# facebookresearch/dmc-net

Measured on AMD Instinct MI355X. Metric: clips/sec (3-seg 224x224) DMC-gen+ResNet-18 train step, higher is better.
Workload: dtype f32

## Files before the change

dmc-net_amd/csrc/conv_x3q.hip:

```cpp
#include "dmc_common.h"
#include "x3s_common.h"
#include <type_traits>
#include <utility>

using namespace dmc;
using namespace dmc::x3;

namespace {

constexpr int QBM = 256, QBN = 64;
constexpr int QWSLOT = 3 * QBN * 32;
constexpr int QWB = 3 * QWSLOT;
constexpr int QEP = 272, QETILE = 32 * QEP;

template <int NW_, int NPB_, int NT_>
struct QG {
    static constexpr int NW = NW_, NPB = NPB_, NT = NT_;
    static constexpr int NA = NW / 2;
    static constexpr int KP = (NT + NA - 1) / NA;
    static constexpr int PT = 3 * KP;
    static constexpr int KW = (18 + NA - 1) / NA;
    static constexpr int ZROW = 32 * NT;
    static constexpr int PSL = (ZROW + 1) * 32;
    static constexpr int PB = 3 * PSL;
// ... 165 lines not shown
            if (U < total_units) {
#pragma unroll
                for (int i = 0; i < QPT; ++i) dma_patch(U / NUNIT, std::integral_constant<int, U % NUNIT>{}, U, i);
            }
        });
    } else {
        static_for<2>([&](auto gc) {
            constexpr int g = decltype(gc)::value;
            if (g < total_steps) {
#pragma unroll
                for (int i = 0; i < KW; ++i) dma_weight(g / NSTEP, std::integral_constant<int, g % NSTEP>{}, g, wq + NA * i);
            }
        });
    }
    asm volatile("s_waitcnt vmcnt(0)" ::: "memory");
    __builtin_amdgcn_s_barrier();

    Frag F0, F1;
    int pb = 0, wb = 0;
    int xcur[NSH];
#pragma unroll
    for (int sh = 0; sh < NSH; ++sh) xcur[sh] = xaddr[sh];
    int wcur = waddr;
    {
        constexpr int sh0 = P::STEP[0].s[0].sh;
        load_frags(F0, xcur[sh0], wcur, std::integral_constant<int, 0>{});
    }

    auto frag_of = [&](auto ic) -> Frag& {
        if constexpr (decltype(ic)::value == 0) return F0; else return F1;
    };
#pragma unroll 1
    for (int c = 0; c < nchunk; ++c) {
        static_for<NSTEP>([&](auto jc) {
            constexpr int J = decltype(jc)::value;
            constexpr int JN = (J + 1) % NSTEP;
            constexpr int unit = P::STEP[J].unit, nslot = P::STEP[J].nslot;
            constexpr bool unit_last = (P::STEP[JN].unit != unit) || (NUNIT == 1 && J == NSTEP - 1);
            constexpr int par = slots_before<P>(J) & 1;
            const int g = c * NSTEP + J, U = c * NUNIT + unit;
            static_for<nslot - 1>([&](auto kc) {
                constexpr int k = decltype(kc)::value;
                constexpr int sh_next = P::STEP[J].s[k + 1].sh, acc_k = P::STEP[J].s[k].acc;
                load_frags(frag_of(std::integral_constant<int, (par + k + 1) & 1>{}), xcur[sh_next], wcur, std::integral_constant<int, k + 1>{});
                mfma_slot(frag_of(std::integral_constant<int, (par + k) & 1>{}), std::integral_constant<int, acc_k>{}, nothing);
                interleave();
            });
            if (GEO::COUNTED && grp_a && U + 2 < total_units) asm volatile("s_waitcnt vmcnt(%0) lgkmcnt(0)" :: "n"(QPT) : "memory");
            else asm volatile("s_waitcnt vmcnt(0) lgkmcnt(0)" ::: "memory");
            __builtin_amdgcn_s_barrier();
            const int pb_old = pb, wb_old = wb;
            if constexpr (unit_last) {
                pb = pb == QNPB - 1 ? 0 : pb + 1;
#pragma unroll
                for (int sh = 0; sh < NSH; ++sh) xcur[sh] = xaddr[sh] + pb * QPB;
            }
            wb ^= 1;
            wcur = waddr + wb * QWB;
            constexpr int kl = nslot - 1;
            constexpr int sh_first = P::STEP[JN].s[0].sh, acc_last = P::STEP[J].s[kl].acc;
            if (g + 1 < total_steps)
                load_frags(frag_of(std::integral_constant<int, (par + kl + 1) & 1>{}), xcur[sh_first], wcur, std::integral_constant<int, 0>{});
            constexpr int J2 = (J + 2) % NSTEP, C2 = (J + 2) / NSTEP;
            constexpr int U3 = (unit + QNPB) % NUNIT, CU3 = (unit + QNPB) / NUNIT;
            const bool wgo = !grp_a && g + 2 < total_steps;
            const bool pgo = grp_a && unit_last && U + QNPB < total_units;
            mfma_slot(frag_of(std::integral_constant<int, (par + kl) & 1>{}), std::integral_constant<int, acc_last>{}, [&](int p) {
                if (wgo) {
#pragma unroll
                    for (int i = p; i < KW; i += 6) dma_weight(c + C2, std::integral_constant<int, J2>{}, wb_old, wq + NA * i);
                }
                if constexpr (unit_last) {
                    if (pgo) {
#pragma unroll
                        for (int i = p; i < QPT; i += 6) dma_patch(c + CU3, std::integral_constant<int, U3>{}, pb_old, i);
                    }
                }
            });
        });
    }

    __syncthreads();
    constexpr int CW = 32 * TN, LPR = CW / 4, RPI = 64 / LPR;
    char* etile = lds_q + wave * QETILE;
    const int mw0 = m0 + wm * 32;
    const int rbase = blockIdx.y * QBN + wn * CW;
    const bool ok = mw0 + l31 <= mlast;
#pragma unroll
    for (int A = 0; A < NACC; ++A) {
#pragma unroll
        for (int j = 0; j < TN; ++j)
#pragma unroll
            for (int g4 = 0; g4 < 4; ++g4) {
                float4 v = make_float4(acc[A][j][4 * g4], acc[A][j][4 * g4 + 1], acc[A][j][4 * g4 + 2], acc[A][j][4 * g4 + 3]);
                if (!ok) v = make_float4(0.f, 0.f, 0.f, 0.f);
                *reinterpret_cast<float4*>(etile + l31 * QEP + (32 * j + 8 * g4 + 4 * khalf) * 4) = v;
            }
        float* const yout = (NACC == 2 && A == 1) ? a.y1 : a.y0;
#pragma unroll
        for (int it = 0; it < 32 / RPI; ++it) {
            const int prow = RPI * it + lane / LPR;
            const int m = mw0 + prow;
            const float4 v = *reinterpret_cast<const float4*>(etile + prow * QEP + (lane % LPR) * 16);
            if (m <= mlast) {
                size_t opix = (size_t)m;
                if (NACC == 4) {
                    const int n = m / HW, rem = m - n * HW, ya = rem / a.W, xb = rem - ya * a.W;
                    opix = ((size_t)n * (2 * a.H) + 2 * ya + (A >> 1)) * (2 * a.W) + 2 * xb + (A & 1);
                }
                *reinterpret_cast<float4*>(yout + opix * a.R + rbase + (lane % LPR) * 4) = v;
            }
        }
        if (NACC == 2) {
            double* const part = A == 1 ? a.part1 : a.part0;
            if (part) {
                double* red = reinterpret_cast<double*>(lds_q + QNW * QETILE);
                if (lane < CW) {
                    double d1 = 0.0, d2 = 0.0;
#pragma unroll 8
                    for (int p = 0; p < 32; ++p) {
                        const double v = (double)*reinterpret_cast<const float*>(etile + p * QEP + lane * 4);
                        d1 += v;
                        d2 += v * v;
                    }
                    red[(wm * 64 + wn * CW + lane) * 2 + 0] = d1;
                    red[(wm * 64 + wn * CW + lane) * 2 + 1] = d2;
                }
                __syncthreads();
                for (int cc = tid; cc < QBN; cc += QNW * 64) {
                    double e1 = 0.0, e2 = 0.0;
#pragma unroll
                    for (int w = 0; w < WM; ++w) { e1 += red[(w * 64 + cc) * 2 + 0]; e2 += red[(w * 64 + cc) * 2 + 1]; }
                    double* dst = part + ((size_t)blockIdx.x * a.R + blockIdx.y * QBN + cc) * 2;
                    dst[0] = e1; dst[1] = e2;
                }
                __syncthreads();
            }
        }
    }
}

__global__ __launch_bounds__(256) void x3q_pack_w_kernel(const float* __restrict__ w3, const float* __restrict__ w1,
                                                         unsigned short* __restrict__ wf, unsigned short* __restrict__ wt, int Cout, int Cin) {
    const bool transposed = blockIdx.y == 1;
    unsigned short* dst = transposed ? wt : wf;
    if (!dst) return;
    const int R = transposed ? Cin : Cout, K = transposed ? Cout : Cin;
    const int nchunk = K >> 4;
    const long total = (long)R * 10 * K;
    for (long i = (long)blockIdx.x * 256 + threadIdx.x; i < total; i += (long)gridDim.x * 256) {
        long t = i;
        const int kk = (int)(t & 15); t >>= 4;
        const int rl = (int)(t & 63); t >>= 6;
        const int slot = (int)(t % 10); t /= 10;
        const int ch = (int)(t % nchunk);
        const int rt = (int)(t / nchunk);
        const int r = rt * 64 + rl, k = ch * 16 + kk;
        constexpr int FWD_TAP[10] = {0, 2, 6, 8, 3, 5, 1, 7, 4, 9};
        const int tap = transposed ? slot : FWD_TAP[slot];
        const int co = transposed ? k : r, ci = transposed ? r : k;
        const float v = tap < 9 ? w3[((long)co * 9 + tap) * Cin + ci] : w1[(long)co * Cin + ci];
        unsigned u0, u1, u2;
        split3(v, u0, u1, u2);
        const size_t base = ((((size_t)(rt * nchunk + ch) * 10 + slot) * 3) * 64 + rl) * 16 + (kk ^ (((rl >> 3) & 1) << 3));
        dst[base] = (unsigned short)(u0 >> 16);
        dst[base + 64 * 16] = (unsigned short)(u1 >> 16);
        dst[base + 2 * 64 * 16] = (unsigned short)(u2 >> 16);
    }
}

__global__ __launch_bounds__(256) void x3q_split_kernel(const float* __restrict__ x, unsigned short* __restrict__ xq, int N, int H, int W, int C) {
    const int c8 = C >> 3, nchunk = C >> 4, H2 = H >> 1, W2 = W >> 1;
    const long total = (long)N * H * W * c8;
    const size_t Mq = (size_t)N * H2 * W2;
    for (long o = (long)blockIdx.x * 256 + threadIdx.x; o < total; o += (long)gridDim.x * 256) {
        const long m = o / c8;
        const int g = (int)(o - m * c8);
        const int xx = (int)(m % W), yy = (int)((m / W) % H), n = (int)(m / ((long)W * H));
        const float4 a = reinterpret_cast<const float4*>(x)[2 * o], b = reinterpret_cast<const float4*>(x)[2 * o + 1];
        const float v[8] = {a.x, a.y, a.z, a.w, b.x, b.y, b.z, b.w};
        const int cls = (yy & 1) * 2 + (xx & 1);
        x3s_store8(xq, v, Mq, 4 * nchunk, ((size_t)n * H2 + (yy >> 1)) * W2 + (xx >> 1), g + cls * 2 * nchunk);
    }
}

__global__ __launch_bounds__(256) void x3q_merge_kernel(const unsigned short* __restrict__ xq, float* __restrict__ x, int N, int H, int W, int C) {
    const int nchunk = C >> 4, H2 = H >> 1, W2 = W >> 1;
    const long total = (long)N * H * W * C;
    const size_t Mq = (size_t)N * H2 * W2, plane = Mq * 16;
    for (long o = (long)blockIdx.x * 256 + threadIdx.x; o < total; o += (long)gridDim.x * 256) {
        const long m = o / C;
        const int c = (int)(o - m * C);
        const int xx = (int)(m % W), yy = (int)((m / W) % H), n = (int)(m / ((long)W * H));
        const int cls = (yy & 1) * 2 + (xx & 1);
        const size_t mq = ((size_t)n * H2 + (yy >> 1)) * W2 + (xx >> 1);
        const size_t w = ((size_t)(cls * nchunk + (c >> 4)) * Mq + mq) * 16 + (c & 15);
        const float s0 = __uint_as_float((unsigned)xq[w] << 16);
        const float s1 = __uint_as_float((unsigned)xq[(size_t)4 * nchunk * plane + w] << 16);
        const float s2 = __uint_as_float((unsigned)xq[(size_t)8 * nchunk * plane + w] << 16);
        x[o] = (s0 + s1) + s2;
    }
}

int stream_blocks_q(long total) {
    long b = (total + 255) / 256;
    return (int)(b < 1 ? 1 : (b > 8192 ? 8192 : b));
}

int q_patch_pixels_max(long M, int W) {
// ... 488 lines not shown
```

dmc-net_amd/csrc/conv_x3s.hip:

```cpp
#include "dmc_common.h"
#include "x3s_common.h"
#include <type_traits>

using namespace dmc;
using namespace dmc::x3;

namespace {

__global__ __launch_bounds__(256) void x3s_split_kernel(const float* __restrict__ x, unsigned short* __restrict__ xs, long M, int C) {
    const int c8 = C >> 3;
    const long total = M * c8;
    const int nchunk = C >> 4;
    for (long o = (long)blockIdx.x * 256 + threadIdx.x; o < total; o += (long)gridDim.x * 256) {
        const long m = o / c8;
        const int g = (int)(o - m * c8);
        const float4 a = reinterpret_cast<const float4*>(x)[2 * o], b = reinterpret_cast<const float4*>(x)[2 * o + 1];
        const float v[8] = {a.x, a.y, a.z, a.w, b.x, b.y, b.z, b.w};
        x3s_store8(xs, v, (size_t)M, nchunk, (size_t)m, g);
    }
}

__global__ __launch_bounds__(256) void x3s_merge_kernel(const unsigned short* __restrict__ xs, float* __restrict__ x, long M, int C) {
    const long total = M * C;
    const size_t plane = (size_t)M * 16;
    const int nchunk = C >> 4;
    for (long o = (long)blockIdx.x * 256 + threadIdx.x; o < total; o += (long)gridDim.x * 256) {
        const long m = o / C;
        const int c = (int)(o - m * C);
        const size_t w = ((size_t)(c >> 4) * M + m) * 16 + (c & 15);
        const float a = __uint_as_float((unsigned)xs[w] << 16);
        const float b = __uint_as_float((unsigned)xs[(size_t)nchunk * plane + w] << 16);
        const float d = __uint_as_float((unsigned)xs[(size_t)2 * nchunk * plane + w] << 16);
        x[o] = (a + b) + d;
    }
}

__global__ __launch_bounds__(256) void x3s_pack_w_kernel(const float* __restrict__ w, unsigned short* __restrict__ wf,
                                                         unsigned short* __restrict__ wt, int Cout, int Cin, int mirror) {
    const bool transposed = blockIdx.y == 1;
    unsigned short* dst = transposed ? wt : wf;
    if (!dst) return;
    const int R = transposed ? Cin : Cout, K = transposed ? Cout : Cin;
    const int nchunk = K >> 4;
    const long total = (long)R * 9 * K;
    for (long i = (long)blockIdx.x * 256 + threadIdx.x; i < total; i += (long)gridDim.x * 256) {
        long t = i;
        const int kk = (int)(t & 15); t >>= 4;
        const int rl = (int)(t & 63); t >>= 6;
        const int tap = (int)(t % 9); t /= 9;
        const int ch = (int)(t % nchunk);
        const int rt = (int)(t / nchunk);
        const int r = rt * 64 + rl, k = ch * 16 + kk;
        const float v = transposed ? w[((long)k * 9 + (mirror ? 8 - tap : tap)) * Cin + r] : w[((long)r * 9 + tap) * Cin + k];
        unsigned u0, u1, u2;
        split3(v, u0, u1, u2);
        const size_t base = ((((size_t)(rt * nchunk + ch) * 9 + tap) * 3) * 64 + rl) * 16 + (kk ^ (((rl >> 3) & 1) << 3));
        dst[base] = (unsigned short)(u0 >> 16);
        dst[base + 64 * 16] = (unsigned short)(u1 >> 16);
        dst[base + 2 * 64 * 16] = (unsigned short)(u2 >> 16);
    }
}

struct X3Args {
    const void* xs;
    const void* wp;
    float* y;
    const float* addend;
    double* stat_part;
    int N, H, W, K, R;
    int M;
    unsigned plane_bytes;
    const float* bnb_y = nullptr;
    const float* bnb_stats = nullptr;
    const float* bnb_gamma = nullptr;
    const float* bnb_beta = nullptr;
    const unsigned char* bnb_mask = nullptr;
    int bnb_relu = 0;
    double* bnb_part = nullptr;
    int part_blocks = -1;
    int ablate;
};

template <int WM, int WN, int TM, int TN, int PPMAX, bool STAG = false, int CLS = 1>
__global__ __launch_bounds__(WM * WN * 64) void x3s_conv_kernel(X3Args a) {
    constexpr int NW = WM * WN, BM = 32 * TM * WM, BN = 32 * TN * WN;
    static_assert(BN == 64, "packed weight image is 64 rows wide");
    static_assert(PPMAX % 32 == 0 || PPMAX % 32 == 1, "patch transfers move 32 pixel rows");
    constexpr int PSL = PPMAX * 32;
    constexpr int PB = 3 * PSL;
    constexpr int WB = 3 * 3 * BN * 32;
    constexpr int WOFF = 2 * PB;
    static_assert(!STAG || NW >= 4, "two transfer groups need four waves");
    constexpr int NA = STAG ? NW / 2 : NW, NB = NW - (STAG ? NA : 0);
    constexpr int NDW = (PPMAX / 32 + NA - 1) / NA;
    constexpr int NEW = WB / 1024;
    constexpr int NEWW = (NEW + NB - 1) / NB;
    extern __shared__ __attribute__((aligned(1024))) char lds_x3[];

    const int tid = threadIdx.x, lane = tid & 63;
    const int wave = __builtin_amdgcn_readfirstlane(tid >> 6);
    const int wm = wave % WM, wn = wave / WM;
    const int l31 = lane & 31, khalf = lane >> 5;
    const unsigned lds0 = lds_addr_of(lds_x3);

    const int HW = a.H * a.W, PW = a.W;
    constexpr int ZROW = PPMAX - 1;
    const int m0 = blockIdx.x * BM;
    const int mlast = (m0 + BM < a.M ? m0 + BM : a.M) - 1;
    const int r_first = m0 / PW, r_last = mlast / PW;
    const int f0 = (r_first > 0 ? r_first - 1 : 0) * PW;
    const int f1 = (r_last + 2) * PW < a.M ? (r_last + 2) * PW : a.M;
    const int PP = f1 - f0;
    const int ND = (PP + 31) >> 5;

    unsigned pvoff[NDW];
#pragma unroll
    for (int k = 0; k < NDW; ++k) {
        const int pr = 32 * (wave + NA * k) + (lane >> 1), h = lane & 1;
        pvoff[k] = pr < PP ? (unsigned)(f0 + pr) * 32u + (unsigned)((h ^ ((pr >> 3) & 1)) << 4) : OOB;
    }
    int xaddr[TM][9];
#pragma unroll
    for (int i = 0; i < TM; ++i) {
        int m = m0 + (wm * TM + i) * 32 + l31;
        if (m > mlast) m = mlast;
        const int n = m / HW, rem = m - n * HW, yy = rem / a.W, xx = rem - yy * a.W;
        const int pp = m - f0;
#pragma unroll
        for (int t = 0; t < 9; ++t) {
            const int dx = CLS == 4 ? (t % 3 == 0 ? 1 : 0) : t % 3 - 1, dy = CLS == 4 ? (t / 3 == 0 ? 1 : 0) : t / 3 - 1;
            const int row = (xx + dx >= 0 && xx + dx < a.W && yy + dy >= 0 && yy + dy < a.H) ? pp + dy * PW + dx : ZROW;
            xaddr[i][t] = row * 32 + ((khalf ^ ((row >> 3) & 1)) << 4);
        }
    }
    const int waddr = (wn * TN * 32 + l31) * 32 + ((khalf ^ ((l31 >> 3) & 1)) << 4);

    const u32x4 srd_x = make_srd(a.xs);
    const int nchunk = a.K >> 4, S = 3 * nchunk;
    const u32x4 srd_w = make_srd(reinterpret_cast<const char*>(a.wp) + (size_t)blockIdx.y * S * WB);
    const unsigned lane16 = (unsigned)lane * 16u;

    const bool grp_a = wave < NA, grp_b = !STAG || wave >= NA;
    const int wb = STAG ? wave - NA : wave;
    auto dma_weight = [&](int step, int wbuf, int k) {
        const int e = wb + NB * k;
        if (e < NEW) dma_buf16(srd_w, lane16, (unsigned)(step * WB + e * 1024), lds0 + WOFF + wbuf * WB + e * 1024);
    };
    auto dma_patch = [&](int chunk, int slice, int pbuf, int k) {
        const int d = wave + NA * k;
        if (d < ND) dma_buf16(srd_x, pvoff[k], (unsigned)(slice * nchunk + chunk) * a.plane_bytes, lds0 + pbuf * PB + slice * PSL + d * 1024);
    };
    auto issue_weights = [&](int step, int wbuf) {
        if (grp_b) {
#pragma unroll
            for (int k = 0; k < NEWW; ++k) dma_weight(step, wbuf, k);
        }
    };
    auto issue_patch = [&](int chunk, int slice, int pbuf) {
        if (grp_a) {
#pragma unroll
            for (int k = 0; k < NDW; ++k) dma_patch(chunk, slice, pbuf, k);
        }
    };

    f32x16 acc[CLS][TM][TN];
#pragma unroll
// ... 40 lines not shown
        for (int k = 0; k < NRD; ++k) {
            __builtin_amdgcn_sched_group_barrier(0x008, 1, 0);
            __builtin_amdgcn_sched_group_barrier(0x100, 1, 0);
        }
        __builtin_amdgcn_sched_group_barrier(0x008, NMF - NRD, 0);
    };
    const bool dma_on = !(DMC_ABL(a.ablate) & 64);
    auto step = [&](auto pbufc, auto wbufc, auto qc, Frag& FA, Frag& FB, int c) {
        constexpr int pbuf = decltype(pbufc)::value, wbuf = decltype(wbufc)::value, q = decltype(qc)::value;
        using NP = std::integral_constant<int, q == 2 ? (pbuf ^ 1) : pbuf>;
        using NWB = std::integral_constant<int, wbuf ^ 1>;
        using NT = std::integral_constant<int, q == 2 ? 0 : 3 * (q + 1)>;
        using T0 = std::integral_constant<int, 3 * q>;
        using T1 = std::integral_constant<int, 3 * q + 1>;
        using T2 = std::integral_constant<int, 3 * q + 2>;
        const int s = 3 * c + q;
        load_frags(pbufc, wbufc, std::integral_constant<int, 3 * q + 1>{}, FB);
        if constexpr (STAG) {
            const bool go = grp_b && dma_on && s + 1 < S;
            mfma_frags(FA, T0{}, [&](int p) {
                if (go) {
#pragma unroll
                    for (int k = p; k < NEWW; k += 6) dma_weight(s + 1, wbuf ^ 1, k);
                }
            });
        } else {
            mfma_frags(FA, T0{}, nothing);
            interleave();
        }
        load_frags(pbufc, wbufc, std::integral_constant<int, 3 * q + 2>{}, FA);
        mfma_frags(FB, T1{}, nothing);
        interleave();
        if (DMC_ABL(a.ablate) & 16) asm volatile("s_waitcnt lgkmcnt(0)" ::: "memory");
        else asm volatile("s_waitcnt vmcnt(0) lgkmcnt(0)" ::: "memory");
        __builtin_amdgcn_s_barrier();
        const int vc = q == 2 ? c + 2 : c + 1;
        if constexpr (STAG) {
            if (s + 1 < S) load_frags(NP{}, NWB{}, NT{}, FB);
            const bool go = grp_a && dma_on && vc < nchunk;
            mfma_frags(FA, T2{}, [&](int p) {
                if (go) {
#pragma unroll
                    for (int k = p; k < NDW; k += 6) dma_patch(vc, q == 2 ? 0 : q + 1, q == 2 ? pbuf : (pbuf ^ 1), k);
                }
            });
        } else {
            if (dma_on) {
                if (s + 2 < S) issue_weights(s + 2, wbuf);
                if (vc < nchunk) issue_patch(vc, q == 2 ? 0 : q + 1, q == 2 ? pbuf : (pbuf ^ 1));
            }
            if (s + 1 < S) load_frags(NP{}, NWB{}, NT{}, FB);
            mfma_frags(FA, T2{}, nothing);
        }
    };
    using I0 = std::integral_constant<int, 0>;
    using I1 = std::integral_constant<int, 1>;
    using Q0 = std::integral_constant<int, 0>;
    using Q1 = std::integral_constant<int, 1>;
    using Q2 = std::integral_constant<int, 2>;

    if (tid < 12)
        *reinterpret_cast<float4*>(lds_x3 + (tid >> 1) * PSL + ZROW * 32 + (tid & 1) * 16) = make_float4(0.f, 0.f, 0.f, 0.f);
    issue_weights(0, 0);
    issue_patch(0, 0, 0); issue_patch(0, 1, 0); issue_patch(0, 2, 0);
    asm volatile("s_waitcnt vmcnt(0)" ::: "memory");
    __builtin_amdgcn_s_barrier();
    if (dma_on) {
        if (!STAG && S > 1) issue_weights(1, 1);
        if (nchunk > 1) issue_patch(1, 0, 1);
    }
    Frag F0, F1;
    load_frags(I0{}, I0{}, Q0{}, F0);
#pragma unroll 1
    for (int c = 0; c < ((DMC_ABL(a.ablate) & 256) ? 0 : nchunk); c += 2) {
        step(I0{}, I0{}, Q0{}, F0, F1, c);
        step(I0{}, I1{}, Q1{}, F1, F0, c);
        step(I0{}, I0{}, Q2{}, F0, F1, c);
        step(I1{}, I1{}, Q0{}, F1, F0, c + 1);
        step(I1{}, I0{}, Q1{}, F0, F1, c + 1);
        step(I1{}, I1{}, Q2{}, F1, F0, c + 1);
    }

    static_assert(WN == 1 && TN == 2, "epilogue: a wave owns all 64 channels of its pixels");
    constexpr int EP = 272, ETILE = 32 * TM * EP;
    char* etile = lds_x3 + wave * ETILE;
    const int mw0 = m0 + wm * TM * 32;
    const int rbase = blockIdx.y * BN;
#pragma unroll
    for (int cl = 0; cl < CLS; ++cl) {
#pragma unroll
        for (int i = 0; i < TM; ++i) {
            const bool ok = mw0 + 32 * i + l31 <= mlast;
#pragma unroll
            for (int j = 0; j < TN; ++j)
#pragma unroll
                for (int g = 0; g < 4; ++g) {
                    float4 v = make_float4(acc[cl][i][j][4 * g], acc[cl][i][j][4 * g + 1], acc[cl][i][j][4 * g + 2], acc[cl][i][j][4 * g + 3]);
                    if (!ok) v = make_float4(0.f, 0.f, 0.f, 0.f);
                    *reinterpret_cast<float4*>(etile + (32 * i + l31) * EP + (32 * j + 8 * g + 4 * khalf) * 4) = v;
                }
        }
        if (!(DMC_ABL(a.ablate) & 128)) {
#pragma unroll
            for (int it = 0; it < 8 * TM; ++it) {
                const int prow = 4 * it + (lane >> 4);
                const int m = mw0 + prow;
                float4 v = *reinterpret_cast<const float4*>(etile + prow * EP + (lane & 15) * 16);
                if (m <= mlast) {
                    size_t opix = (size_t)m;
                    if (CLS == 4) {
                        const int n = m / HW, rem = m - n * HW, ya = rem / a.W, xb = rem - ya * a.W;
                        opix = ((size_t)n * (2 * a.H) + 2 * ya + (cl >> 1)) * (2 * a.W) + 2 * xb + (cl & 1);
                    }
                    const size_t o = opix * a.R + rbase + (lane & 15) * 4;
                    if (a.addend) {
                        const float4 av = *reinterpret_cast<const float4*>(a.addend + o);
                        v.x += av.x; v.y += av.y; v.z += av.z; v.w += av.w;
                    }
                    *reinterpret_cast<float4*>(a.y + o) = v;
                    if (CLS == 1 && a.bnb_part) {
                        const int c4 = rbase + (lane & 15) * 4;
                        const float4 yv = *reinterpret_cast<const float4*>(a.bnb_y + o);
                        const float4 mean = *reinterpret_cast<const float4*>(a.bnb_stats + c4);
                        const float4 istd = *reinterpret_cast<const float4*>(a.bnb_stats + a.R + c4);
                        const float4 xh = make_float4((yv.x - mean.x) * istd.x, (yv.y - mean.y) * istd.y, (yv.z - mean.z) * istd.z, (yv.w - mean.w) * istd.w);
                        if (a.bnb_relu) {
                            unsigned mb;
                            if (a.bnb_mask) {
                                mb = a.bnb_mask[o >> 2];
                            } else {
                                const float4 g = *reinterpret_cast<const float4*>(a.bnb_gamma + c4), b = *reinterpret_cast<const float4*>(a.bnb_beta + c4);
                                mb = (fmaf(xh.x, g.x, b.x) > 0.f ? 1u : 0u) | (fmaf(xh.y, g.y, b.y) > 0.f ? 2u : 0u) |
                                     (fmaf(xh.z, g.z, b.z) > 0.f ? 4u : 0u) | (fmaf(xh.w, g.w, b.w) > 0.f ? 8u : 0u);
                            }
                            v.x = (mb & 1) ? v.x : 0.f; v.y = (mb & 2) ? v.y : 0.f; v.z = (mb & 4) ? v.z : 0.f; v.w = (mb & 8) ? v.w : 0.f;
                        }
                        *reinterpret_cast<float4*>(etile + prow * EP + (lane & 15) * 16) = v;
                        *reinterpret_cast<float4*>(etile + NW * ETILE + 8192 + prow * EP + (lane & 15) * 16) = xh;
                    }
                } else if (CLS == 1 && a.bnb_part) {
                    *reinterpret_cast<float4*>(etile + prow * EP + (lane & 15) * 16) = make_float4(0.f, 0.f, 0.f, 0.f);
                    *reinterpret_cast<float4*>(etile + NW * ETILE + 8192 + prow * EP + (lane & 15) * 16) = make_float4(0.f, 0.f, 0.f, 0.f);
                }
            }
        }
    }
    if (CLS == 1 && a.bnb_part) {
        double* red = reinterpret_cast<double*>(lds_x3 + NW * ETILE);
        const char* xtile = etile + NW * ETILE + 8192;
        double d1 = 0.0, d2 = 0.0;
#pragma unroll 8
        for (int p = 0; p < 32 * TM; ++p) {
            const double d = (double)*reinterpret_cast<const float*>(etile + p * EP + lane * 4);
            const double xh = (double)*reinterpret_cast<const float*>(xtile + p * EP + lane * 4);
            d1 += d;
            d2 += d * xh;
        }
        red[(wm * 64 + lane) * 2 + 0] = d1;
        red[(wm * 64 + lane) * 2 + 1] = d2;
        __syncthreads();
        for (int cc = tid; cc < BN; cc += NW * 64) {
            double e1 = 0.0, e2 = 0.0;
#pragma unroll
            for (int w = 0; w < WM; ++w) { e1 += red[(w * 64 + cc) * 2 + 0]; e2 += red[(w * 64 + cc) * 2 + 1]; }
            double* dst = a.bnb_part + ((size_t)blockIdx.x * a.R + rbase + cc) * 2;
            dst[0] = e1; dst[1] = e2;
        }
    }
    if (CLS == 1 && a.stat_part) {
        double* red = reinterpret_cast<double*>(lds_x3 + NW * ETILE);
        double d1 = 0.0, d2 = 0.0;
#pragma unroll 8
        for (int p = 0; p < 32 * TM; ++p) {
            const double v = (double)*reinterpret_cast<const float*>(etile + p * EP + lane * 4);
            d1 += v;
            d2 += v * v;
        }
        red[(wm * 64 + lane) * 2 + 0] = d1;
        red[(wm * 64 + lane) * 2 + 1] = d2;
        __syncthreads();
        for (int c = tid; c < BN; c += NW * 64) {
            double e1 = 0.0, e2 = 0.0;
#pragma unroll
            for (int w = 0; w < WM; ++w) { e1 += red[(w * 64 + c) * 2 + 0]; e2 += red[(w * 64 + c) * 2 + 1]; }
            double* dst = a.stat_part + ((size_t)blockIdx.x * a.R + rbase + c) * 2;
            dst[0] = e1; dst[1] = e2;
        }
    }
}

int patch_pixels_max(int N, int H, int W, int BM) {
    const long M = (long)N * H * W;
    int worst = 0;
    long tiles = (M + BM - 1) / BM;
    if (tiles > W) tiles = W;
    for (long t = 0; t < tiles; ++t) {
        const long m0 = t * BM, ml = (m0 + BM < M ? m0 + BM : M) - 1;
        const long r0 = m0 / W, r1 = ml / W;
        const long f0 = (r0 > 0 ? r0 - 1 : 0) * W, f1 = (r1 + 2) * W;
        if ((int)(f1 - f0) + 1 > worst) worst = (int)(f1 - f0) + 1;
    }
    return worst;
}

struct X3Cfg { int id, BM, PPMAX, threads; };
constexpr X3Cfg X3CFGS[] = {{0, 256, 608, 512}, {1, 128, 320, 256}, {2, 64, 192, 128}, {3, 256, 608, 256}, {4, 128, 225, 256}};

bool x3s_shape_ok(int N, int H, int W, int K, int R) {
    if (N <= 0 || H <= 0 || W <= 0 || K % 32 != 0 || R % 64 != 0 || K <= 0 || R <= 0) return false;
    const long M = (long)N * H * W;
    return M * (K > R ? K : R) * 6 < (1L << 31);
}

int x3s_choose(int N, int H, int W, int R) {
    const long M = (long)N * H * W;
    const int forced = option(OPT_CONV_CFG);
    if (forced >= 101 && forced <= 105 && patch_pixels_max(N, H, W, X3CFGS[forced - 101].BM) <= X3CFGS[forced - 101].PPMAX) return forced - 101;
    if (forced != 106 && patch_pixels_max(N, H, W, X3CFGS[4].BM) <= X3CFGS[4].PPMAX && ((M + X3CFGS[4].BM - 1) / X3CFGS[4].BM) * (R / 64) >= 512)
        return 4;
    int fallback = -1;
    for (const X3Cfg& c : X3CFGS) {
        if (c.id > 2 || patch_pixels_max(N, H, W, c.BM) > c.PPMAX) continue;
        const long wgs = ((M + c.BM - 1) / c.BM) * (R / 64);
        if (wgs >= 160) return c.id;
        fallback = c.id;
    }
    return fallback;
}

template <int WM, int TM, int PPMAX>
int launch_x3s(const X3Args& a, hipStream_t s) {
    constexpr int BM = 32 * TM * WM;
    constexpr size_t op_bytes = 2 * 3 * PPMAX * 32 + 2 * 3 * 3 * 64 * 32, ep_bytes = 2 * (size_t)BM * 272 + 8192;
    constexpr size_t lds_bytes = op_bytes > ep_bytes ? op_bytes : ep_bytes;
    dim3 grid((a.M + BM - 1) / BM, a.R / 64);
    if ((a.stat_part || a.bnb_part) && a.part_blocks >= 0 && (unsigned)a.part_blocks != grid.x)
        return fail(DMC_E_INVALID, "x3s_conv: statistics partials have %d rows but this launch writes %u (dmc_x3s_conv_stat_blocks was "
                                   "called under another conv_cfg option?)", a.part_blocks, grid.x);
    if constexpr (WM >= 4) {
        if (!(option(OPT_CONV_ABLATE) & 512)) {
            static LdsLimit lim_attr2;
    const hipError_t attr2 = lim_attr2.raise(reinterpret_cast<const void*>(&x3s_conv_kernel<WM, 1, TM, 2, PPMAX, true>), (int)lds_bytes);
            if (attr2 != hipSuccess) return fail(DMC_E_LAUNCH, "x3s_conv: cannot raise the dynamic LDS limit: %s", hipGetErrorString(attr2));
            x3s_conv_kernel<WM, 1, TM, 2, PPMAX, true><<<grid, WM * 64, lds_bytes, s>>>(a);
            return check_launch("x3s_conv");
        }
    }
    static LdsLimit lim_attr;
    const hipError_t attr = lim_attr.raise(reinterpret_cast<const void*>(&x3s_conv_kernel<WM, 1, TM, 2, PPMAX>), (int)lds_bytes);
    if (attr != hipSuccess) return fail(DMC_E_LAUNCH, "x3s_conv: cannot raise the dynamic LDS limit: %s", hipGetErrorString(attr));
    x3s_conv_kernel<WM, 1, TM, 2, PPMAX><<<grid, WM * 64, lds_bytes, s>>>(a);
    return check_launch("x3s_conv");
}

struct X3Bnb { const float *y, *stats, *gamma, *beta; const unsigned char* mask; int relu; double* part; };

int run_x3s(const void* xs, const void* wp, const float* addend, float* y, double* stat_part, int part_blocks, int N, int H, int W,
            int K, int R, hipStream_t s, const X3Bnb* bnb = nullptr) {
    if (!xs || !wp || !y) return fail(DMC_E_INVALID, "x3s_conv: null pointer");
    if (!x3s_shape_ok(N, H, W, K, R)) return fail(DMC_E_INVALID, "x3s_conv: unsupported shape N=%d H=%d W=%d K=%d R=%d", N, H, W, K, R);
    const int cfg = x3s_choose(N, H, W, R);
    X3Args a;
    a.xs = xs; a.wp = wp; a.y = y; a.addend = addend; a.stat_part = stat_part;
    a.N = N; a.H = H; a.W = W; a.K = K; a.R = R; a.M = N * H * W;
    a.plane_bytes = (unsigned)a.M * 32u;
    a.part_blocks = part_blocks;
    if ((stat_part || bnb) && part_blocks <= 0) return fail(DMC_E_INVALID, "x3s_conv: stat_blocks must be the row count of the partials");
    if (bnb) {
        a.bnb_y = bnb->y; a.bnb_stats = bnb->stats; a.bnb_gamma = bnb->gamma; a.bnb_beta = bnb->beta; a.bnb_mask = bnb->mask;
        a.bnb_relu = bnb->relu; a.bnb_part = bnb->part;
    }
    a.ablate = option(OPT_CONV_ABLATE);
    if (DMC_ABL(a.ablate) & 32) a.stat_part = nullptr;
    switch (cfg) {
        case 0: return launch_x3s<8, 1, 608>(a, s);
        case 1: return launch_x3s<4, 1, 320>(a, s);
        case 2: return launch_x3s<2, 1, 192>(a, s);
        case 3: return launch_x3s<4, 2, 608>(a, s);
        case 4: return launch_x3s<4, 1, 225>(a, s);
        default: return fail(DMC_E_INVALID, "x3s_conv: the patch of a %d x %d image does not fit the LDS", H, W);
    }
}

struct X3WgArgs {
    const void* xs;
    const void* dys;
    float* part;
    int N, H, Cin, Cout;
    unsigned plane_bytes;
    int steps, per_group, tiles_ci;
};

template <int W_, int R>
struct WgGeom {
    static constexpr int PW = W_ + 2;
    static constexpr int NGRP = R >= W_ + 2 ? 2 : 4, LA = NGRP / 2;
    static constexpr int NRING = NGRP * R;
    static constexpr int XPX = NRING * PW;
    static constexpr int XPL = ((XPX + 3) / 8) * 8 + 4;
    static constexpr int NPX = R * W_;
    static constexpr int NKB = (NPX + 15) / 16;
    static constexpr int DYP = NKB * 16;
    static constexpr int DYT = ((DYP + 31) / 32) * 32;
    static constexpr int DYPL = ((DYT + 3) / 8) * 8 + 4;
    static constexpr int XI = (R * PW + 31) / 32;
    static constexpr int DI = DYT / 32;
    static constexpr int XBYTES = 12 * XPL * 32, DYBYTES = 12 * DYPL * 32;
    static constexpr int LDS = XBYTES + 2 * DYBYTES;
};

template <int W_, int R>
__global__ __launch_bounds__(768) void x3s_wgrad_kernel(X3WgArgs a) {
    using G = WgGeom<W_, R>;
    constexpr int PW = G::PW, NRING = G::NRING, XPL = G::XPL, DYPL = G::DYPL, NKB = G::NKB;
    extern __shared__ __attribute__((aligned(1024))) char lds_wg[];
    const int tid = threadIdx.x, lane = tid & 63;
    const int wave = __builtin_amdgcn_readfirstlane(tid >> 6);
    const int l31 = lane & 31, khalf = lane >> 5, L = lane & 15, grp = (lane >> 4) & 1;
    const int quarter = wave & 3, trow = wave >> 2;
    const int wi = quarter & 1, wj = quarter >> 1;
    const int tci = blockIdx.x % a.tiles_ci, tco = blockIdx.x / a.tiles_ci;
    const unsigned lds0 = lds_addr_of(lds_wg);
    const int HP = a.H + 2;
    const int s_begin = blockIdx.y * a.per_group;
    const int s_end = s_begin + a.per_group < a.steps ? s_begin + a.per_group : a.steps;
    const u32x4 srd_x = make_srd(a.xs), srd_d = make_srd(a.dys);
    const unsigned soff_x = (unsigned)((wave >> 2) * (a.Cin >> 4) + tci * 4 + (wave & 3)) * a.plane_bytes;
    const unsigned soff_d = (unsigned)((wave >> 2) * (a.Cout >> 4) + tco * 4 + (wave & 3)) * a.plane_bytes;
    const unsigned xplane = lds0 + (unsigned)wave * XPL * 32, dplane = lds0 + G::XBYTES + (unsigned)wave * DYPL * 32;
    const int lpx = lane >> 1;
    const unsigned lhalf = (unsigned)(lane & 1) << 4;

    const unsigned img_bytes = (unsigned)(a.H * W_) * 32u;
    unsigned xpre[G::XI], dpre[G::DI];
#pragma unroll
    for (int i = 0; i < G::XI; ++i) {
        const int px = 32 * i + lpx;
        const int r = px / PW, col = px - r * PW - 1;
        xpre[i] = (col >= 0 && col < W_) ? (unsigned)(r * W_ + col) * 32u + lhalf : NOPIX;
    }
#pragma unroll
    for (int i = 0; i < G::DI; ++i) {
        const int p = 32 * i + lpx;
        dpre[i] = p < G::NPX ? (unsigned)p * 32u + lhalf : NOPIX;
    }
    auto issue_x = [&](int q, const WgGroupPos& g) {
        const int slot0 = (((q % G::NGRP) + G::NGRP) % G::NGRP) * R;
        unsigned tbase, img_off;
        wg_group_base(g, a.N, W_, img_bytes, tbase, img_off);
#pragma unroll
        for (int i = 0; i < G::XI; ++i)
            if (32 * i + lpx < R * PW)
                dma_buf16(srd_x, wg_lane_off(tbase, xpre[i], img_bytes), soff_x + img_off, xplane + (unsigned)(slot0 * PW + 32 * i) * 32u);
    };
    auto issue_dy = [&](const WgGroupPos& g, int buf) {
        unsigned tbase, img_off;
        wg_group_base(g, a.N, W_, img_bytes, tbase, img_off);
#pragma unroll
        for (int i = 0; i < G::DI; ++i)
            dma_buf16(srd_d, wg_lane_off(tbase, dpre[i], img_bytes), soff_d + img_off, dplane + (unsigned)buf * G::DYBYTES + (unsigned)(32 * i) * 32u);
    };

// ... 285 lines not shown
```

dmc-net_amd/csrc/x3s_common.h:

```cpp
#pragma once
#include "dmc_common.h"

namespace dmc {
namespace x3 {

typedef float f32x16 __attribute__((ext_vector_type(16)));
typedef __bf16 bf16x8 __attribute__((ext_vector_type(8)));
typedef unsigned u32x4 __attribute__((ext_vector_type(4)));
typedef const __attribute__((address_space(3))) char* lds_cptr;

__device__ __forceinline__ f32x16 mfma_bf16(const u32x4& a, const u32x4& b, const f32x16& c) {
    return __builtin_amdgcn_mfma_f32_32x32x16_bf16(__builtin_bit_cast(bf16x8, a), __builtin_bit_cast(bf16x8, b), c, 0, 0, 0);
}

__device__ __forceinline__ void split3(float v, unsigned& u0, unsigned& u1, unsigned& u2) {
    u0 = __float_as_uint(v);
    const float r1 = v - __uint_as_float(u0 & 0xffff0000u);
    u1 = __float_as_uint(r1);
    u2 = __float_as_uint(r1 - __uint_as_float(u1 & 0xffff0000u));
}
__device__ __forceinline__ unsigned pack_hi(unsigned hi_of_second, unsigned hi_of_first) {
    return __builtin_amdgcn_perm(hi_of_second, hi_of_first, 0x07060302u);
}

constexpr unsigned OOB = 0x80000000u;

__device__ __forceinline__ void dma_buf16(const u32x4& srd, unsigned voff, unsigned soff, unsigned lds_byte_addr) {
    asm volatile("s_mov_b32 m0, %2\n\ts_nop 3\n\tbuffer_load_dwordx4 %0, %1, %3 offen lds"
                 :: "v"(voff), "s"(srd), "s"(lds_byte_addr), "s"(soff) : "memory");
}
__device__ __forceinline__ u32x4 make_srd(const void* base) {
    const unsigned long long b = (unsigned long long)base;
    u32x4 srd;
    srd[0] = __builtin_amdgcn_readfirstlane((unsigned)b);
    srd[1] = __builtin_amdgcn_readfirstlane((unsigned)(b >> 32) & 0xffffu);
    srd[2] = 0x7fffffffu;
    srd[3] = 0x00020000u;
    return srd;
}

typedef short s16x4 __attribute__((ext_vector_type(4)));
__device__ __forceinline__ void tr_read2(lds_cptr p0, lds_cptr p1, u32x4& f) {
    const s16x4 a = __builtin_amdgcn_ds_read_tr16_b64_v4i16((__attribute__((address_space(3))) s16x4*)p0);
    const s16x4 b = __builtin_amdgcn_ds_read_tr16_b64_v4i16((__attribute__((address_space(3))) s16x4*)p1);
    typedef unsigned u32x2 __attribute__((ext_vector_type(2)));
    const u32x2 ua = __builtin_bit_cast(u32x2, a), ub = __builtin_bit_cast(u32x2, b);
    f[0] = ua[0]; f[1] = ua[1]; f[2] = ub[0]; f[3] = ub[1];
}

constexpr unsigned NOPIX = 0x40000000u;

struct WgGroupPos { int n, y; };
__device__ __forceinline__ WgGroupPos wg_group_at(int q, int R, int HP) {
    const int g = R * q, n = g / HP;
    WgGroupPos p;
    p.n = __builtin_amdgcn_readfirstlane(n);
    p.y = __builtin_amdgcn_readfirstlane(g - n * HP);
    return p;
}
__device__ __forceinline__ WgGroupPos wg_group_next(WgGroupPos p, int R, int HP) {
    p.y += R;
    if (p.y >= HP) { p.y -= HP; ++p.n; }
    return p;
}
__device__ __forceinline__ WgGroupPos wg_group_prev(WgGroupPos p, int R, int HP) {
    p.y -= R;
    if (p.y < 0) { p.y += HP; --p.n; }
    return p;
}
__device__ __forceinline__ void wg_group_base(const WgGroupPos& p, int N, int W, unsigned img_bytes, unsigned& tbase, unsigned& img_off) {
    const bool in = p.n >= 0 && p.n < N;
    tbase = in ? (unsigned)((p.y - 1) * W) * 32u : NOPIX;
    img_off = in ? (unsigned)p.n * img_bytes : 0u;
}
__device__ __forceinline__ unsigned wg_lane_off(unsigned tbase, unsigned pre, unsigned img_bytes) {
    const unsigned t = tbase + pre;
    return t < img_bytes ? t : OOB;
}

typedef float f32x4 __attribute__((ext_vector_type(4)));
__device__ __forceinline__ f32x4 mfma16(const u32x4& a, const u32x4& b, const f32x4& c) {
    return __builtin_amdgcn_mfma_f32_16x16x32_bf16(__builtin_bit_cast(bf16x8, a), __builtin_bit_cast(bf16x8, b), c, 0, 0, 0);
}

__device__ __forceinline__ void split8(const float4& lo, const float4& hi, u32x4& s0, u32x4& s1, u32x4& s2) {
    const float v[8] = {lo.x, lo.y, lo.z, lo.w, hi.x, hi.y, hi.z, hi.w};
    unsigned u0[8], u1[8], u2[8];
#pragma unroll
    for (int e = 0; e < 8; ++e) split3(v[e], u0[e], u1[e], u2[e]);
#pragma unroll
    for (int e = 0; e < 4; ++e) {
        s0[e] = pack_hi(u0[2 * e + 1], u0[2 * e]);
        s1[e] = pack_hi(u1[2 * e + 1], u1[2 * e]);
        s2[e] = pack_hi(u2[2 * e + 1], u2[2 * e]);
    }
}

}
}
```

Before: 3586.

## Accumulate BatchNorm column sums in registers during conv epilogue writeback

Replaces the per-column LDS re-read loop that computed channel sum and sum-of-squares (or the BN-backward dot terms) with per-lane double accumulators filled while the epilogue writes outputs, followed by a small in-wave LDS combine. Adds a compile-time BNB template variant so the upstream BatchNorm backward fusion prefetches y and mask values before the epilogue and no longer stages masked gradients and xhat in a second LDS tile. This halves the epilogue LDS reservation. The costs are more register pressure from the prefetched arrays and double accumulators, plus extra kernel instantiations.

```diff
diff --git a/dmc-net_amd/csrc/conv_x3q.hip b/dmc-net_amd/csrc/conv_x3q.hip
--- a/dmc-net_amd/csrc/conv_x3q.hip
+++ b/dmc-net_amd/csrc/conv_x3q.hip
@@ -271,6 +271,7 @@
 
     __syncthreads();
     constexpr int CW = 32 * TN, LPR = CW / 4, RPI = 64 / LPR;
+    static_assert(QETILE >= 4096, "ColSums::wave_total needs 4 KB of the wave's tile");
     char* etile = lds_q + wave * QETILE;
     const int mw0 = m0 + wm * 32;
     const int rbase = blockIdx.y * QBN + wn * CW;
@@ -286,11 +287,17 @@
                 *reinterpret_cast<float4*>(etile + l31 * QEP + (32 * j + 8 * g4 + 4 * khalf) * 4) = v;
             }
         float* const yout = (NACC == 2 && A == 1) ? a.y1 : a.y0;
+        double* const part = NACC == 2 ? (A == 1 ? a.part1 : a.part0) : nullptr;
+        ColSums cs;
+        cs.clear();
 #pragma unroll
         for (int it = 0; it < 32 / RPI; ++it) {
             const int prow = RPI * it + lane / LPR;
             const int m = mw0 + prow;
             const float4 v = *reinterpret_cast<const float4*>(etile + prow * QEP + (lane % LPR) * 16);
+            if (NACC == 2) {
+                if (part) cs.add(v, v);
+            }
             if (m <= mlast) {
                 size_t opix = (size_t)m;
                 if (NACC == 4) {
@@ -301,19 +308,12 @@
             }
         }
         if (NACC == 2) {
-            double* const part = A == 1 ? a.part1 : a.part0;
             if (part) {
                 double* red = reinterpret_cast<double*>(lds_q + QNW * QETILE);
-                if (lane < CW) {
-                    double d1 = 0.0, d2 = 0.0;
-#pragma unroll 8
-                    for (int p = 0; p < 32; ++p) {
-                        const double v = (double)*reinterpret_cast<const float*>(etile + p * QEP + lane * 4);
-                        d1 += v;
-                        d2 += v * v;
-                    }
-                    red[(wm * 64 + wn * CW + lane) * 2 + 0] = d1;
-                    red[(wm * 64 + wn * CW + lane) * 2 + 1] = d2;
+                double t1, t2;
+                if (cs.template wave_total<CW>(etile, lane, t1, t2)) {
+                    red[(wm * 64 + wn * CW + lane) * 2 + 0] = t1;
+                    red[(wm * 64 + wn * CW + lane) * 2 + 1] = t2;
                 }
                 __syncthreads();
                 for (int cc = tid; cc < QBN; cc += QNW * 64) {
diff --git a/dmc-net_amd/csrc/conv_x3s.hip b/dmc-net_amd/csrc/conv_x3s.hip
--- a/dmc-net_amd/csrc/conv_x3s.hip
+++ b/dmc-net_amd/csrc/conv_x3s.hip
@@ -81,7 +81,7 @@
     int ablate;
 };
 
-template <int WM, int WN, int TM, int TN, int PPMAX, bool STAG = false, int CLS = 1>
+template <int WM, int WN, int TM, int TN, int PPMAX, bool STAG = false, int CLS = 1, bool BNB = false>
 __global__ __launch_bounds__(WM * WN * 64) void x3s_conv_kernel(X3Args a) {
     constexpr int NW = WM * WN, BM = 32 * TM * WM, BN = 32 * TN * WN;
     static_assert(BN == 64, "packed weight image is 64 rows wide");
@@ -288,10 +288,33 @@
     }
 
     static_assert(WN == 1 && TN == 2, "epilogue: a wave owns all 64 channels of its pixels");
+    static_assert(!BNB || CLS == 1, "upstream BatchNorm sums: stride-1 data gradient only");
     constexpr int EP = 272, ETILE = 32 * TM * EP;
+    static_assert(ETILE >= 4096, "ColSums::wave_total needs 4 KB of the wave's tile");
     char* etile = lds_x3 + wave * ETILE;
     const int mw0 = m0 + wm * TM * 32;
     const int rbase = blockIdx.y * BN;
+    const int c4 = rbase + (lane & 15) * 4;
+    constexpr int NIT = 8 * TM;
+    float4 by[BNB ? NIT : 1];
+    unsigned bm[BNB ? NIT : 1];
+    if constexpr (BNB) {
+        const bool masked = a.bnb_relu && a.bnb_mask;
+#pragma unroll
+        for (int it = 0; it < NIT; ++it) {
+            const int m = mw0 + 4 * it + (lane >> 4);
+            by[it] = make_float4(0.f, 0.f, 0.f, 0.f);
+            bm[it] = 0u;
+            if (m <= mlast) {
+                const size_t o = (size_t)m * a.R + c4;
+                by[it] = *reinterpret_cast<const float4*>(a.bnb_y + o);
+                if (masked) bm[it] = a.bnb_mask[o >> 2];
+            }
+        }
+    }
+    ColSums cs;
+    cs.clear();
+    const bool want_stat = CLS == 1 && !BNB && a.stat_part;
 #pragma unroll
     for (int cl = 0; cl < CLS; ++cl) {
 #pragma unroll
@@ -307,11 +330,23 @@
                 }
         }
         if (!(DMC_ABL(a.ablate) & 128)) {
-#pragma unroll
-            for (int it = 0; it < 8 * TM; ++it) {
+            float4 bmean = make_float4(0.f, 0.f, 0.f, 0.f), bistd = bmean, bgam = bmean, bbet = bmean;
+            if constexpr (BNB) {
+                bmean = *reinterpret_cast<const float4*>(a.bnb_stats + c4);
+                bistd = *reinterpret_cast<const float4*>(a.bnb_stats + a.R + c4);
+                if (a.bnb_relu && !a.bnb_mask) {
+                    bgam = *reinterpret_cast<const float4*>(a.bnb_gamma + c4);
+                    bbet = *reinterpret_cast<const float4*>(a.bnb_beta + c4);
+                }
+            }
+#pragma unroll
+            for (int it = 0; it < NIT; ++it) {
                 const int prow = 4 * it + (lane >> 4);
                 const int m = mw0 + prow;
                 float4 v = *reinterpret_cast<const float4*>(etile + prow * EP + (lane & 15) * 16);
+                if (CLS == 1 && !BNB) {
+                    if (want_stat) cs.add(v, v);
+                }
                 if (m <= mlast) {
                     size_t opix = (size_t)m;
                     if (CLS == 4) {
@@ -324,73 +359,40 @@
                         v.x += av.x; v.y += av.y; v.z += av.z; v.w += av.w;
                     }
                     *reinterpret_cast<float4*>(a.y + o) = v;
-                    if (CLS == 1 && a.bnb_part) {
-                        const int c4 = rbase + (lane & 15) * 4;
-                        const float4 yv = *reinterpret_cast<const float4*>(a.bnb_y + o);
-                        const float4 mean = *reinterpret_cast<const float4*>(a.bnb_stats + c4);
-                        const float4 istd = *reinterpret_cast<const float4*>(a.bnb_stats + a.R + c4);
-                        const float4 xh = make_float4((yv.x - mean.x) * istd.x, (yv.y - mean.y) * istd.y, (yv.z - mean.z) * istd.z, (yv.w - mean.w) * istd.w);
+                    if constexpr (BNB) {
+                        const float4 yv = by[it];
+                        const float4 xh = make_float4((yv.x - bmean.x) * bistd.x, (yv.y - bmean.y) * bistd.y, (yv.z - bmean.z) * bistd.z,
+                                                      (yv.w - bmean.w) * bistd.w);
                         if (a.bnb_relu) {
-                            unsigned mb;
-                            if (a.bnb_mask) {
-                                mb = a.bnb_mask[o >> 2];
-                            } else {
-                                const float4 g = *reinterpret_cast<const float4*>(a.bnb_gamma + c4), b = *reinterpret_cast<const float4*>(a.bnb_beta + c4);
-                                mb = (fmaf(xh.x, g.x, b.x) > 0.f ? 1u : 0u) | (fmaf(xh.y, g.y, b.y) > 0.f ? 2u : 0u) |
-                                     (fmaf(xh.z, g.z, b.z) > 0.f ? 4u : 0u) | (fmaf(xh.w, g.w, b.w) > 0.f ? 8u : 0u);
-                            }
+                            unsigned mb = bm[it];
+                            if (!a.bnb_mask)
+                                mb = (fmaf(xh.x, bgam.x, bbet.x) > 0.f ? 1u : 0u) | (fmaf(xh.y, bgam.y, bbet.y) > 0.f ? 2u : 0u) |
+                                     (fmaf(xh.z, bgam.z, bbet.z) > 0.f ? 4u : 0u) | (fmaf(xh.w, bgam.w, bbet.w) > 0.f ? 8u : 0u);
                             v.x = (mb & 1) ? v.x : 0.f; v.y = (mb & 2) ? v.y : 0.f; v.z = (mb & 4) ? v.z : 0.f; v.w = (mb & 8) ? v.w : 0.f;
                         }
-                        *reinterpret_cast<float4*>(etile + prow * EP + (lane & 15) * 16) = v;
-                        *reinterpret_cast<float4*>(etile + NW * ETILE + 8192 + prow * EP + (lane & 15) * 16) = xh;
+                        cs.add(v, xh);
                     }
-                } else if (CLS == 1 && a.bnb_part) {
-                    *reinterpret_cast<float4*>(etile + prow * EP + (lane & 15) * 16) = make_float4(0.f, 0.f, 0.f, 0.f);
-                    *reinterpret_cast<float4*>(etile + NW * ETILE + 8192 + prow * EP + (lane & 15) * 16) = make_float4(0.f, 0.f, 0.f, 0.f);
                 }
             }
         }
     }
-    if (CLS == 1 && a.bnb_part) {
-        double* red = reinterpret_cast<double*>(lds_x3 + NW * ETILE);
-        const char* xtile = etile + NW * ETILE + 8192;
-        double d1 = 0.0, d2 = 0.0;
-#pragma unroll 8
-        for (int p = 0; p < 32 * TM; ++p) {
-            const double d = (double)*reinterpret_cast<const float*>(etile + p * EP + lane * 4);
-            const double xh = (double)*reinterpret_cast<const float*>(xtile + p * EP + lane * 4);
-            d1 += d;
-            d2 += d * xh;
-        }
-        red[(wm * 64 + lane) * 2 + 0] = d1;
-        red[(wm * 64 + lane) * 2 + 1] = d2;
-        __syncthreads();
-        for (int cc = tid; cc < BN; cc += NW * 64) {
-            double e1 = 0.0, e2 = 0.0;
-#pragma unroll
-            for (int w = 0; w < WM; ++w) { e1 += red[(w * 64 + cc) * 2 + 0]; e2 += red[(w * 64 + cc) * 2 + 1]; }
-            double* dst = a.bnb_part + ((size_t)blockIdx.x * a.R + rbase + cc) * 2;
-            dst[0] = e1; dst[1] = e2;
-        }
-    }
-    if (CLS == 1 && a.stat_part) {
-        double* red = reinterpret_cast<double*>(lds_x3 + NW * ETILE);
-        double d1 = 0.0, d2 = 0.0;
-#pragma unroll 8
-        for (int p = 0; p < 32 * TM; ++p) {
-            const double v = (double)*reinterpret_cast<const float*>(etile + p * EP + lane * 4);
-            d1 += v;
-            d2 += v * v;
-        }
-        red[(wm * 64 + lane) * 2 + 0] = d1;
-        red[(wm * 64 + lane) * 2 + 1] = d2;
-        __syncthreads();
-        for (int c = tid; c < BN; c += NW * 64) {
-            double e1 = 0.0, e2 = 0.0;
-#pragma unroll
-            for (int w = 0; w < WM; ++w) { e1 += red[(w * 64 + c) * 2 + 0]; e2 += red[(w * 64 + c) * 2 + 1]; }
-            double* dst = a.stat_part + ((size_t)blockIdx.x * a.R + rbase + c) * 2;
-            dst[0] = e1; dst[1] = e2;
+    if constexpr (CLS == 1) {
+        double* const part = BNB ? a.bnb_part : a.stat_part;
+        if (BNB || want_stat) {
+            double* red = reinterpret_cast<double*>(lds_x3 + NW * ETILE);
+            double t1, t2;
+            if (cs.template wave_total<64>(etile, lane, t1, t2)) {
+                red[(wm * 64 + lane) * 2 + 0] = t1;
+                red[(wm * 64 + lane) * 2 + 1] = t2;
+            }
+            __syncthreads();
+            for (int c = tid; c < BN; c += NW * 64) {
+                double e1 = 0.0, e2 = 0.0;
+#pragma unroll
+                for (int w = 0; w < WM; ++w) { e1 += red[(w * 64 + c) * 2 + 0]; e2 += red[(w * 64 + c) * 2 + 1]; }
+                double* dst = part + ((size_t)blockIdx.x * a.R + rbase + c) * 2;
+                dst[0] = e1; dst[1] = e2;
+            }
         }
     }
 }
@@ -434,10 +436,10 @@
     return fallback;
 }
 
-template <int WM, int TM, int PPMAX>
+template <int WM, int TM, int PPMAX, bool BNB = false>
 int launch_x3s(const X3Args& a, hipStream_t s) {
     constexpr int BM = 32 * TM * WM;
-    constexpr size_t op_bytes = 2 * 3 * PPMAX * 32 + 2 * 3 * 3 * 64 * 32, ep_bytes = 2 * (size_t)BM * 272 + 8192;
+    constexpr size_t op_bytes = 2 * 3 * PPMAX * 32 + 2 * 3 * 3 * 64 * 32, ep_bytes = (size_t)BM * 272 + 8192;
     constexpr size_t lds_bytes = op_bytes > ep_bytes ? op_bytes : ep_bytes;
     dim3 grid((a.M + BM - 1) / BM, a.R / 64);
     if ((a.stat_part || a.bnb_part) && a.part_blocks >= 0 && (unsigned)a.part_blocks != grid.x)
@@ -446,16 +448,16 @@
     if constexpr (WM >= 4) {
         if (!(option(OPT_CONV_ABLATE) & 512)) {
             static LdsLimit lim_attr2;
-    const hipError_t attr2 = lim_attr2.raise(reinterpret_cast<const void*>(&x3s_conv_kernel<WM, 1, TM, 2, PPMAX, true>), (int)lds_bytes);
+    const hipError_t attr2 = lim_attr2.raise(reinterpret_cast<const void*>(&x3s_conv_kernel<WM, 1, TM, 2, PPMAX, true, 1, BNB>), (int)lds_bytes);
             if (attr2 != hipSuccess) return fail(DMC_E_LAUNCH, "x3s_conv: cannot raise the dynamic LDS limit: %s", hipGetErrorString(attr2));
-            x3s_conv_kernel<WM, 1, TM, 2, PPMAX, true><<<grid, WM * 64, lds_bytes, s>>>(a);
+            x3s_conv_kernel<WM, 1, TM, 2, PPMAX, true, 1, BNB><<<grid, WM * 64, lds_bytes, s>>>(a);
             return check_launch("x3s_conv");
         }
     }
     static LdsLimit lim_attr;
-    const hipError_t attr = lim_attr.raise(reinterpret_cast<const void*>(&x3s_conv_kernel<WM, 1, TM, 2, PPMAX>), (int)lds_bytes);
+    const hipError_t attr = lim_attr.raise(reinterpret_cast<const void*>(&x3s_conv_kernel<WM, 1, TM, 2, PPMAX, false, 1, BNB>), (int)lds_bytes);
     if (attr != hipSuccess) return fail(DMC_E_LAUNCH, "x3s_conv: cannot raise the dynamic LDS limit: %s", hipGetErrorString(attr));
-    x3s_conv_kernel<WM, 1, TM, 2, PPMAX><<<grid, WM * 64, lds_bytes, s>>>(a);
+    x3s_conv_kernel<WM, 1, TM, 2, PPMAX, false, 1, BNB><<<grid, WM * 64, lds_bytes, s>>>(a);
     return check_launch("x3s_conv");
 }
 
@@ -478,12 +480,13 @@
     }
     a.ablate = option(OPT_CONV_ABLATE);
     if (DMC_ABL(a.ablate) & 32) a.stat_part = nullptr;
+    const bool nb = a.bnb_part != nullptr;
     switch (cfg) {
-        case 0: return launch_x3s<8, 1, 608>(a, s);
-        case 1: return launch_x3s<4, 1, 320>(a, s);
-        case 2: return launch_x3s<2, 1, 192>(a, s);
-        case 3: return launch_x3s<4, 2, 608>(a, s);
-        case 4: return launch_x3s<4, 1, 225>(a, s);
+        case 0: return nb ? launch_x3s<8, 1, 608, true>(a, s) : launch_x3s<8, 1, 608>(a, s);
+        case 1: return nb ? launch_x3s<4, 1, 320, true>(a, s) : launch_x3s<4, 1, 320>(a, s);
+        case 2: return nb ? launch_x3s<2, 1, 192, true>(a, s) : launch_x3s<2, 1, 192>(a, s);
+        case 3: return nb ? launch_x3s<4, 2, 608, true>(a, s) : launch_x3s<4, 2, 608>(a, s);
+        case 4: return nb ? launch_x3s<4, 1, 225, true>(a, s) : launch_x3s<4, 1, 225>(a, s);
         default: return fail(DMC_E_INVALID, "x3s_conv: the patch of a %d x %d image does not fit the LDS", H, W);
     }
 }
diff --git a/dmc-net_amd/csrc/x3s_common.h b/dmc-net_amd/csrc/x3s_common.h
--- a/dmc-net_amd/csrc/x3s_common.h
+++ b/dmc-net_amd/csrc/x3s_common.h
@@ -47,6 +47,40 @@
     const u32x2 ua = __builtin_bit_cast(u32x2, a), ub = __builtin_bit_cast(u32x2, b);
     f[0] = ua[0]; f[1] = ua[1]; f[2] = ub[0]; f[3] = ub[1];
 }
+
+struct ColSums {
+    double s[4], q[4];
+    __device__ __forceinline__ void clear() {
+#pragma unroll
+        for (int e = 0; e < 4; ++e) s[e] = q[e] = 0.0;
+    }
+    __device__ __forceinline__ void add(const float4& a, const float4& b) {
+        const float av[4] = {a.x, a.y, a.z, a.w}, bv[4] = {b.x, b.y, b.z, b.w};
+#pragma unroll
+        for (int e = 0; e < 4; ++e) {
+            s[e] += (double)av[e];
+            q[e] = __builtin_fma((double)av[e], (double)bv[e], q[e]);
+        }
+    }
+    template <int CW>
+    __device__ __forceinline__ bool wave_total(char* scratch, int lane, double& t1, double& t2) const {
+        constexpr int NG = 256 / CW;
+        double2* comb = reinterpret_cast<double2*>(scratch);
+#pragma unroll
+        for (int e = 0; e < 4; ++e) comb[4 * lane + e] = make_double2(s[e], q[e]);
+        __builtin_amdgcn_wave_barrier();
+        if (lane >= CW) return false;
+        double2 t = comb[lane];
+#pragma unroll
+        for (int g = 1; g < NG; ++g) {
+            const double2 u = comb[g * CW + lane];
+            t.x += u.x;
+            t.y += u.y;
+        }
+        t1 = t.x; t2 = t.y;
+        return true;
+    }
+};
 
 constexpr unsigned NOPIX = 0x40000000u;
 
```

Result: no change. 3603, median of 6 (+0.5%).
